# Michaelszeng/GCS-ADMM

Hardware: AMD Instinct MI355X
Metric: admm_iterations_per_sec (higher is better)
Workload: dtype f64; 1 GPU; benchmark4; V=42, E=94, n=2, state_dtype=f64, state_columns=incidence, inner_arithmetic=f64, vertex_program=workgroup, vertex_solves=warm start from the previous iteration's record (csrc/warm_start.h), parallelism=1 GPU

## Files before the change

### gcs_admm_amd/csrc/vertex_wg.h

```cpp
#pragma once
#include <type_traits>

#include "gcs_math.h"
#include "step_args.h"
#include "warm_start.h"

#if defined(__HIP_DEVICE_COMPILE__)
#define WG_DEVICE 1
#else
#define WG_DEVICE 0
#endif

namespace gcs_wg {

using gcs_math::REG_DELTA;
using gcs_math::rcp;
using gcs_math::rcp1;
using gcs_math::rsqrt_nr;
using gcs_math::sqrt_nr;

#ifndef GCS_WG_THREADS
#define GCS_WG_THREADS 256
#endif
constexpr int WG_THREADS = GCS_WG_THREADS;
constexpr int WG_WAVES = WG_THREADS / 64;
constexpr int WG_ITEM_WAVES = WG_WAVES > 1 ? WG_WAVES - 1 : 1;

constexpr bool WG_VM = false;
#if WG_DEVICE
template <bool VM> __device__ __forceinline__ void wg_barrier()
{
    if constexpr (VM) asm volatile("s_waitcnt vmcnt(0)" ::: "memory");
    __syncthreads();
}
template <bool VM> __device__ __forceinline__ void wg_wave_sync()
{
    if constexpr (VM) asm volatile("s_waitcnt vmcnt(0) lgkmcnt(0)" ::: "memory");
    else asm volatile("s_waitcnt lgkmcnt(0)" ::: "memory");
}
__device__ __forceinline__ int wg_tid()
{
    int t = (int)threadIdx.x;
    asm volatile("" : "+v"(t));
    return t;
}
#define WG_FOR(i, cnt) for (int i = gcs_wg::wg_tid(), i##_end = (cnt); i < i##_end; i += gcs_wg::WG_THREADS)
#define WG_FOR_AT(i, cnt, start) for (int i = (gcs_wg::wg_tid() - (start)) & (gcs_wg::WG_THREADS - 1), i##_end = (cnt); i < i##_end; i += gcs_wg::WG_THREADS)
#define WG_SYNC() gcs_wg::wg_barrier<WG_VM>()
#define WG_ONE() if (gcs_wg::wg_tid() == 0)
#define WG_CONE() if (gcs_wg::wg_tid() == gcs_wg::WG_THREADS - 1)
#define WG_CONE2(l) for (int l = gcs_wg::wg_tid() - (gcs_wg::WG_THREADS - 2); l >= 0 && l < 2; l = 2)
#define WG_WAVE0() if (gcs_wg::wg_tid() < 64)
#define WG_FIRST_WAVES(w, cnt) for (int w = gcs_wg::wg_tid() >> 6; w < (cnt); w += gcs_wg::WG_WAVES)
#define WG_ITEM_FOR(q, i, count, PER)                                                                                          \
    for (int t_ = gcs_wg::wg_tid(), w_ = t_ >> 6, l_ = t_ & 63,                                                                \
             n_ = w_ < gcs_wg::WG_ITEM_WAVES ? (((count) - w_ + gcs_wg::WG_ITEM_WAVES - 1) / gcs_wg::WG_ITEM_WAVES) * (PER) : 0;  \
         l_ < n_; l_ += 64)                                                                                                    \
        if (const int qq_ = l_ / (PER), i = l_ - qq_ * (PER), q = w_ + gcs_wg::WG_ITEM_WAVES * qq_; true)
#define WG_REPL_FOR(i, cnt) for (int i = (gcs_wg::wg_tid() >> 6) < gcs_wg::WG_ITEM_WAVES ? (gcs_wg::wg_tid() & 63) : (cnt), i##_end = (cnt); i < i##_end; i += 64)
#define WG_WAVE_SYNC() gcs_wg::wg_wave_sync<WG_VM>()
#define WG_FENCE() asm volatile("" ::: "memory")
#else
#define WG_FENCE() do { } while (0)
#ifdef GCS_WG_REVERSE
#define WG_FOR(i, cnt) for (int i = (cnt) - 1; i >= 0; --i)
#else
#define WG_FOR(i, cnt) for (int i = 0, i##_end = (cnt); i < i##_end; ++i)
#endif
#define WG_FOR_AT(i, cnt, start) WG_FOR(i, ((void)(start), (cnt)))
#define WG_SYNC() do { } while (0)
#define WG_ONE() if (true)
#define WG_CONE() if (true)
#define WG_CONE2(l) for (int l = 0; l < 2; ++l)
#define WG_WAVE0() if (true)
#define WG_FIRST_WAVES(w, cnt) for (int w = 0; w < (cnt); ++w)
#define WG_ITEM_FOR(q, i, count, PER) WG_FOR(t_, (count) * (PER)) if (const int q = t_ / (PER), i = t_ - q * (PER); true)
#define WG_REPL_FOR(i, cnt) WG_FOR(i, cnt)
#define WG_WAVE_SYNC() do { } while (0)
#endif

#if defined(GCS_WG_TIMING) && defined(__HIPCC__)
__device__ unsigned long long g_wg_cycles[64];
__device__ unsigned long long g_wg_counts[64];
__device__ unsigned long long g_wg_wave_cycles[64 * 8];
#endif
#if defined(GCS_WG_TIMING) && WG_DEVICE
__device__ __forceinline__ void wg_stamp(int id, unsigned long long &last)
{
    if (blockIdx.x == 0) {
        const unsigned long long t = __builtin_amdgcn_s_memtime();
        if (threadIdx.x == 0) {
            atomicAdd(&g_wg_cycles[id], t - last);
            atomicAdd(&g_wg_counts[id], 1ull);
        }
        last = t;
    }
}
__device__ __forceinline__ void wg_arrive(int id, unsigned long long last)
{
    if (blockIdx.x == 0) {
        const unsigned long long t = __builtin_amdgcn_s_memtime();
        if ((threadIdx.x & 63) == 0) atomicAdd(&g_wg_wave_cycles[id * 8 + ((threadIdx.x >> 6) & 7)], t - last);
    }
}
#define WG_ARRIVE(id) gcs_wg::wg_arrive(id, wg_last_stamp)
#define WG_STAMP(id) gcs_wg::wg_stamp(id, wg_last_stamp)
#define WG_STAMP_INIT() unsigned long long wg_last_stamp = __builtin_amdgcn_s_memtime()
#else
#define WG_STAMP(id) do { } while (0)
#define WG_ARRIVE(id) do { } while (0)
#define WG_STAMP_INIT() do { } while (0)
#endif

struct Place {
    int off = 0;
    GCS_HD int at(int cnt)
    {
        const int start = off & (WG_THREADS - 1);
        off = (off + cnt + 63) & ~63;
        return start;
    }
};

template <int N> struct WD {
    static constexpr int NW = 2 * N + 1, NX = 2 * N, NB1 = 4 * N + 1, Q = N + 1, NS = N * (N + 1) / 2;
    static constexpr int TA = 2 * NS + 2 * N + 1;
};

constexpr int pad2(int x) { return (x + 1) & ~1; }
template <int N> struct WSoc {
    static constexpr int Q = N + 1;
    static constexpr int SS = 0, LS = Q, WB = 2 * Q, LT = 3 * Q, CV = LT + Q, SU = CV + N, DSSA = SU + N * N, DLSA = DSSA + Q,
                         DSS = DLSA + Q, DLS = DSS + Q, KS = DLS + Q, SIZE = KS + Q;
};
enum { SC_T = 0, SC_DT, SC_DTA, SC_ALPHA, SC_CONEFAIL, SC_C0, SC_ETA, SC_GT, SC_AMAXC, SC_C1C, SC_C2C, SC_AMAXC2, SC_N = 12 };
template <int N> struct WL {
    using D = WD<N>;
    static constexpr int NW = D::NW, NX = D::NX, NB1 = D::NB1;
    static constexpr int CEN = 0, XV = CEN + pad2(N), DX = XV + pad2(NX), NU = DX + pad2(NX), DNU = NU + pad2(2 * NW),
                         BS = DNU + pad2(2 * NW), BSI = BS + pad2(2 * NW * NW), BXS = BSI + pad2(2 * NW * NW),
                         PIVS = BXS + pad2(2 * NW * NX), BG = PIVS + pad2(2 * NW), XBG = BG + pad2(2 * NW), XBX = XBG + pad2(2 * NX),
                         XS = XBX + pad2(2 * NX * NX), RP = XS + pad2(NX * N), VV = RP + pad2(2 * NW), WW = VV + pad2(2 * NW), M = WW + pad2(2 * NW),
                         PIVM = M + pad2(NB1 * NB1), RHS = PIVM + pad2(NB1), SOL = RHS + pad2(NB1),
                         SOC = SOL + pad2(NB1), PQ = SOC + pad2(WSoc<N>::SIZE), PC = PQ + pad2(NX + NW), SC = PC + pad2(NX + NW), RED = SC + pad2(SC_N), FIXED = RED + 3 * 3 * WG_WAVES;
    static constexpr int P = 0, DW = P + pad2(NW), TG = DW + pad2(NW), TF = TG + pad2(NW), LB = TF + pad2(N), KB = LB + 2, DLB = KB + 2,
                         PIV = DLB + 2, G0 = PIV + pad2(NW), GU = G0 + pad2(NW), GX = GU + pad2(NW), TE = GX + pad2(NX),
                         RV = TE + pad2(NW), K = RV + pad2(NW), X = K + pad2(NW * NW), B = X + pad2(NW * NX), ROWS = B + pad2(NW * NW);
    static GCS_HD int unit_stride(int m) { return (ROWS + 12 * m) | 1; }
    static GCS_HD int total(int U, int m) { return FIXED + pad2(U * unit_stride(m)) + pad2(m * N) + pad2(m); }
    static GCS_HD int units_doubles(int U, int m) { return pad2(U * unit_stride(m)); }
};
template <int N> struct WLBox {
    using G = WL<N>;
    using D = WD<N>;
    static constexpr int NW = D::NW, NX = D::NX, NB1 = D::NB1;
    static constexpr int CEN = G::CEN, XV = G::XV, DX = G::DX, NU = G::NU, DNU = G::DNU, BS = G::BS, BSI = G::BSI, BXS = G::BXS, PIVS = G::PIVS,
                         BG = G::BG, XBG = G::XBG, XBX = G::XBX, XS = G::XS, RP = G::RP, VV = G::VV, WW = G::WW, M = G::M, PIVM = G::PIVM,
                         RHS = G::RHS, SOL = G::SOL, SOC = G::SOC, PQ = G::PQ, PC = G::PC, SC = G::SC, RED = G::RED, FIXED = G::FIXED;
    static constexpr int P = G::P, DW = G::DW, TG = G::TG, TF = G::TF, LB = G::LB, KB = G::KB, DLB = G::DLB, G0 = G::G0, GU = G::GU, GX = G::GX,
                         TE = G::TE, RV = G::RV;
    static constexpr int KD = G::K, KY = KD + pad2(NX), KYY = KY + pad2(NX), XD = KYY + 2, XY = XD + pad2(NX),
                         BD = XY + pad2(NX), BW = BD + pad2(NX), BRS = BW + pad2(NW), BQ = BRS + 2, ROWS = BQ + pad2(NX);
    static GCS_HD int unit_stride(int m) { return (ROWS + 12 * m) | 1; }
    static GCS_HD int total(int U, int m) { return FIXED + pad2(U * unit_stride(m)) + pad2(m * N) + pad2(m); }
    static GCS_HD int units_doubles(int U, int m) { return pad2(U * unit_stride(m)); }
};
template <int N> GCS_HD int wg_lds_doubles(int U, int m, bool box = false) { return box ? WLBox<N>::total(U, m) : WL<N>::total(U, m); }
constexpr int WG_MAX_N = 8;
inline bool wg_has_box(int n) { return n == 3 || n == 6; }
inline int wg_lds_doubles_n(int n, int U, int m, bool box = false)
{
    box = box && wg_has_box(n);
    switch (n) {
    case 1: return wg_lds_doubles<1>(U, m);
    case 2: return wg_lds_doubles<2>(U, m);
    case 3: return wg_lds_doubles<3>(U, m, box);
    case 4: return wg_lds_doubles<4>(U, m);
    case 5: return wg_lds_doubles<5>(U, m);
    case 6: return wg_lds_doubles<6>(U, m, box);
    case 7: return wg_lds_doubles<7>(U, m);
    default: return wg_lds_doubles<8>(U, m);
    }
}

struct alignas(8) WgF2 { float a, b; };

template <class T> struct WgArgs : gcsadmm_k::StepArgs<T> {
    int n_vtx;
    const int *vtx;
    const double *prox_q = nullptr, *prox_c = nullptr;
    const int *order = nullptr;
    int *unit_iters = nullptr;
};

struct Red3 { double mn, s1, s2; };

#if WG_DEVICE
template <int SH> __device__ __forceinline__ double dpp_row_shr(double x, double ident)
{
    const int ilo = __double2loint(ident), ihi = __double2hiint(ident);
    const int lo = __builtin_amdgcn_update_dpp(ilo, __double2loint(x), 0x110 + SH, 0xf, 0xf, false);
    const int hi = __builtin_amdgcn_update_dpp(ihi, __double2hiint(x), 0x110 + SH, 0xf, 0xf, false);
    return __hiloint2double(hi, lo);
}
__device__ __forceinline__ double lane_bcast(double x, int lane)
{
    return __hiloint2double(__builtin_amdgcn_readlane(__double2hiint(x), lane), __builtin_amdgcn_readlane(__double2loint(x), lane));
}
#endif

GCS_HD double wg_uniform(double x)
{
#if WG_DEVICE
    return __hiloint2double(__builtin_amdgcn_readfirstlane(__double2hiint(x)), __builtin_amdgcn_readfirstlane(__double2loint(x)));
#else
    return x;
#endif
}
GCS_HD int wg_uniform(int x)
{
#if WG_DEVICE
    return __builtin_amdgcn_readfirstlane(x);
#else
    return x;
#endif
}

template <bool VM = false> GCS_HD Red3 wg_reduce(Red3 v, double *red, int &phase)
{
#if WG_DEVICE
    v.mn = fmin(v.mn, dpp_row_shr<1>(v.mn, 1e300)); v.s1 += dpp_row_shr<1>(v.s1, 0.0); v.s2 += dpp_row_shr<1>(v.s2, 0.0);
    v.mn = fmin(v.mn, dpp_row_shr<2>(v.mn, 1e300)); v.s1 += dpp_row_shr<2>(v.s1, 0.0); v.s2 += dpp_row_shr<2>(v.s2, 0.0);
    v.mn = fmin(v.mn, dpp_row_shr<4>(v.mn, 1e300)); v.s1 += dpp_row_shr<4>(v.s1, 0.0); v.s2 += dpp_row_shr<4>(v.s2, 0.0);
    v.mn = fmin(v.mn, dpp_row_shr<8>(v.mn, 1e300)); v.s1 += dpp_row_shr<8>(v.s1, 0.0); v.s2 += dpp_row_shr<8>(v.s2, 0.0);
    Red3 w;
    w.mn = fmin(fmin(lane_bcast(v.mn, 15), lane_bcast(v.mn, 31)), fmin(lane_bcast(v.mn, 47), lane_bcast(v.mn, 63)));
    w.s1 = (lane_bcast(v.s1, 15) + lane_bcast(v.s1, 31)) + (lane_bcast(v.s1, 47) + lane_bcast(v.s1, 63));
    w.s2 = (lane_bcast(v.s2, 15) + lane_bcast(v.s2, 31)) + (lane_bcast(v.s2, 47) + lane_bcast(v.s2, 63));
    double *buf = red + phase * (3 * WG_WAVES);
    phase = phase == 2 ? 0 : phase + 1;
    const int wave = (int)threadIdx.x >> 6;
    if (((int)threadIdx.x & 63) == 0) { buf[wave * 3 + 0] = w.mn; buf[wave * 3 + 1] = w.s1; buf[wave * 3 + 2] = w.s2; }
    wg_barrier<VM>();
    Red3 r{buf[0], buf[1], buf[2]};
#pragma unroll
    for (int q = 1; q < WG_WAVES; ++q) { r.mn = fmin(r.mn, buf[3 * q]); r.s1 += buf[3 * q + 1]; r.s2 += buf[3 * q + 2]; }
    return r;
#else
    (void)red; (void)phase;
    return v;
#endif
}

GCS_HD void tri_decode(int t, int &r, int &c)
{
    r = (int)((sqrtf(8.0f * (float)t + 1.0f) - 1.0f) * 0.5f);
    if ((r + 1) * (r + 2) / 2 <= t) ++r;
    if (r * (r + 1) / 2 > t) --r;
    c = t - r * (r + 1) / 2;
}

GCS_HD int fdiv(int x, float inv) { return (int)(((float)x + 0.5f) * inv); }

GCS_HD constexpr int pki(int i, int j) { return i * (i + 1) / 2 + j; }

template <int DIM> GCS_HD void wave_ldl(double *Mq, double *rd)
{
    static_assert(DIM <= 64, "one row per lane");
#if WG_DEVICE
    const int lane = wg_tid() & 63, row = lane < DIM ? lane : DIM - 1;
    double a[DIM];
#pragma unroll
    for (int j = 0; j < DIM; ++j) a[j] = Mq[row * DIM + j];
    const double od = Mq[row * DIM + row];
    double myr = 0.0;
#pragma unroll
    for (int k = 0; k < DIM; ++k) {
        const double dk = lane_bcast(a[k], k);
        const double odk = lane_bcast(od, k);
        const double rk = rcp(gcs_math::pivot_floor(dk, odk)), col = a[k], l = col * rk;
        a[k] = l;
        if (lane == k) myr = rk;
#pragma unroll
        for (int j = k + 1; j < DIM; ++j) a[j] -= l * lane_bcast(col, j);
    }
    if (lane < DIM) {
#pragma unroll
        for (int j = 0; j < DIM - 1; ++j) Mq[lane * DIM + j] = a[j];
        rd[lane] = myr;
    }
#else
    double od[DIM], col[DIM];
    for (int k = 0; k < DIM; ++k) od[k] = Mq[k * DIM + k];
    for (int k = 0; k < DIM; ++k) {
        const double rk = rcp(gcs_math::pivot_floor(Mq[k * DIM + k], od[k]));
        rd[k] = rk;
        for (int i = k + 1; i < DIM; ++i) col[i] = Mq[i * DIM + k];
        for (int i = k + 1; i < DIM; ++i) {
            const double l = col[i] * rk;
            Mq[i * DIM + k] = l;
            for (int j = k + 1; j <= i; ++j) Mq[i * DIM + j] -= l * col[j];
        }
    }
#endif
}

template <int DIM> GCS_HD void wave_ldl_solve(const double *Mq, const double *rd, const double *b, double *x)
{
#if WG_DEVICE
    const int lane = wg_tid() & 63, row = lane < DIM ? lane : DIM - 1;
// ... 144 lines not shown
    const int WUS = WR::unit_stride(m);
    double dtm = 0.0;
    Place pl0;
    WG_FOR_AT(t, d * NW, pl0.at(d * NW)) {
        const int e = t / NW, w = t - e * NW, edge = a.inc_edge[lo + e];
        const bool out = e >= d_in;
        const int inc = gcsadmm_k::state_column(a, lo, e, edge, out);
        double *un = UN(e + 1);
        const double Tw = gcsadmm_k::consensus_target(a, w, edge, inc, mu_scale);
        int slot = -1;
        if (w == 2 * N) slot = 2 * N;
        else if (out) slot = w;
        else if (w < N) { un[W::TF + w] = Tw; un[W::TG + N + w] = 0.0; }
        else slot = w - N;
        if (slot >= 0) {
            un[W::TG + slot] = Tw;
            if (wrec) dtm = fmax(dtm, fabs(Tw - wrec[WR::UNITS + (e + 1) * WUS + WR::TG + slot]));
        }
    }
    WG_FOR_AT(t, m * N, pl0.at(m * N)) PA[t] = a.poly_A[(size_t)p0 * N + t];
    WG_FOR_AT(j, m + N, pl0.at(m + N)) {
        if (j < m) PA[pad2(m * N) + j] = a.poly_bc[p0 + j];
        else sm[W::CEN + (j - m)] = a.center[(size_t)v * N + (j - m)];
    }
    if (prox) {
        WG_FOR(k, NX + NW) {
            sm[W::PQ + k] = a.prox_q[(size_t)v * (NX + NW) + k];
            sm[W::PC + k] = a.prox_c[(size_t)v * (NX + NW) + k];
        }
    }
    bool use_warm = false;
    double mu_ref = gcs_ws::WS_COLD_REF, ws_dT = -1.0;
    if (wrec) {
        const Red3 rt = wg_reduce<WG_VM>(Red3{-dtm, 0.0, 0.0}, sm + W::RED, red_phase);
        const bool comparable = wg_uniform((int)(wrec[0] == 1.0 && wrec[1] == rho)) != 0;
        ws_dT = wg_uniform(comparable ? -rt.mn * rho : -1.0);
        use_warm = wg_uniform((int)(comparable && ws_dT <= gcs_ws::ws_theta(wrec))) != 0;
        if (use_warm) mu_ref = wg_uniform(fmax(gcs_ws::WS_MU_MIN, gcs_ws::WS_KAPPA * ws_dT));
    }
    const bool ws_started_warm = use_warm;
    const float inv_R2 = 1.0f / (float)(R / 2);

    WG_STAMP(0);
    auto gval = [&](const double *un, int u, int k, bool wk) {
        double g = un[W::G0 + k];
        if (wk) {
            g += un[W::GU + k];
            if (u == 0 && k < 2 * N) g += k < N ? -SOC[SO::KS + 1 + k] : SOC[SO::KS + 1 + (k - N)];
        }
        return g;
    };
    auto te_tasks = [&](Place &pl, bool wk) {
        WG_FOR_AT(t, d * NW, pl.at(d * NW)) {
            const int u = 1 + t / NW, i = t - (u - 1) * NW;
            double *un = UN(u);
            double s = 0;
            if constexpr (BOX) {
                double wg = 0;
#pragma unroll
                for (int k = 0; k < NW; ++k) wg += un[W::BW + k] * gval(un, u, k, wk);
                s = -(un[W::BRS] * un[W::BW + i]) * wg;
                if (i < 2 * N) s -= un[W::BD + i] * gval(un, u, i, wk);
            } else {
#pragma unroll
                for (int k = 0; k < NW; ++k) s -= un[W::B + i * NW + k] * gval(un, u, k, wk);
            }
            un[W::TE + i] = s;
        }
    };
    auto bg_tasks = [&](Place &pl) {
        WG_FOR_AT(t, 2 * NW, pl.at(2 * NW)) {
            const int s = t / NW, i = t - s * NW;
            double acc = 0;
#pragma unroll 4
            for (int u = side_lo(s); u <= side_hi(s); ++u) acc += UN(u)[W::TE + i];
            sm[W::BG + t] = acc;
        }
        WG_FOR_AT(t, 2 * NX, pl.at(2 * NX)) {
            const int part = t / NX, c = t - part * NX, h = c / N;
            const int ulo = part ? 1 + d / 2 : 1, uhi = part ? d : d / 2;
            double acc = 0;
#pragma unroll 2
            for (int u = ulo; u <= uhi; ++u) {
                const double *un = UN(u);
                if constexpr (BOX) acc += un[W::XD + c] * un[W::TE + c] + un[W::XY + c] * un[W::TE + 2 * N];
                else {
#pragma unroll
                    for (int k = 0; k < N; ++k) acc += un[W::X + (h * N + k) * NX + c] * un[W::TE + h * N + k];
                    acc += un[W::X + 2 * N * NX + c] * un[W::TE + 2 * N];
                }
            }
            sm[W::XBG + t] = acc;
        }
    };
    auto v_tasks = [&](Place &pl) {
        WG_FOR_AT(t, 2 * NW, pl.at(2 * NW)) {
            const int s = t / NW, i = t - s * NW;
            const double *Bsi = sm + W::BSI + s * NW * NW;
            double acc = 0;
#pragma unroll
            for (int k = 0; k < NW; ++k) acc += Bsi[i * NW + k] * (sm[W::RP + s * NW + k] - sm[W::BG + s * NW + k]);
            sm[W::VV + t] = acc;
        }
    };
    auto rhs_tasks = [&](Place &pl, bool wk) {
        const double *u0 = UN(0);
        auto base_z = [&](int i) { return -gval(u0, 0, i, wk) - sm[W::VV + i] - sm[W::VV + NW + i]; };
        WG_FOR_AT(q, NX, pl.at(NX)) {
            double r = -REG_DELTA * sm[W::XV + q] - sm[W::XBG + q] - sm[W::XBG + NX + q];
            if (prox) r -= sm[W::PQ + q] * (sm[W::XV + q] + CEN[q < N ? q : q - N] - sm[W::PC + q]);
            if (wk) r -= sm[W::SOL + q];
            for (int s = 0; s < 2; ++s) {
                const double *BXs = sm + W::BXS + s * NW * NX;
#pragma unroll
                for (int i = 0; i < NW; ++i) r -= BXs[i * NX + q] * sm[W::VV + s * NW + i];
            }
            sm[W::RHS + q] = r;
        }
        WG_FOR_AT(k, N, pl.at(N))
            sm[W::RHS + NX + k] = base_z(k) + SOC[SO::CV + k] * SC[SC_GT] * rcp(SC[SC_C0]);
        WG_FOR_AT(k, N, pl.at(N))
            sm[W::RHS + NX + N + k] = base_z(k) + base_z(N + k);
        WG_FOR_AT(k, 1, pl.at(1)) sm[W::RHS + NX + 2 * N + k] = base_z(2 * N);
    };
    auto solve_head = [&](bool wk) {
        {
            Place pl;
            te_tasks(pl, wk);
            if (wk) {
                WG_FOR_AT(q, NX, pl.at(NX)) {
                    double acc = 0;
#pragma unroll 4
                    for (int u = 0; u <= d; ++u) acc += UN(u)[W::GX + q];
                    sm[W::SOL + q] = acc;
                }
            }
        }
        WG_ARRIVE(30);
        WG_SYNC();
        WG_STAMP(30);
        { Place pl; bg_tasks(pl); }
        WG_ARRIVE(31);
        WG_SYNC();
        WG_STAMP(31);
        { Place pl; v_tasks(pl); }
        WG_ARRIVE(32);
        WG_SYNC();
        WG_STAMP(32);
        { Place pl; rhs_tasks(pl, wk); }
        WG_ARRIVE(33);
        WG_SYNC();
        WG_STAMP(33);
    };
    auto cone_dir = [&](int dt_slot, bool wk, double (&xs)[Q], double (&dl)[Q]) {
        const double *u0 = UN(0);
        double wb[Q], ys[Q];
        xs[0] = SC[dt_slot];
#pragma unroll
        for (int k = 0; k < N; ++k) xs[1 + k] = u0[W::DW + k] - u0[W::DW + N + k];
#pragma unroll
        for (int k = 0; k < Q; ++k) wb[k] = SOC[SO::WB + k];
        soc_apply_W2<Q>(wb, SC[SC_ETA], xs, ys);
#pragma unroll
        for (int k = 0; k < Q; ++k) dl[k] = (wk ? SOC[SO::KS + k] : 0.0) - SOC[SO::LS + k] - ys[k];
    };
    auto solve_tail = [&](int dt_slot, bool wk) {
        WG_WAVE0() wave_ldl_solve<NB1>(sm + W::M, sm + W::PIVM, sm + W::RHS, sm + W::SOL);
        WG_ARRIVE(34);
        WG_SYNC();
        WG_STAMP(34);
        auto dzeta = [&](int i) { return i < N ? sm[W::SOL + NX + i] + sm[W::SOL + NX + N + i] : sm[W::SOL + NX + i]; };
        Place plw;
        WG_FOR_AT(t, 2 * NW, plw.at(2 * NW)) {
            const int s = t / NW, i = t - s * NW;
            const double *BXs = sm + W::BXS + s * NW * NX;
            double acc = dzeta(i) + (sm[W::RP + t] - sm[W::BG + t]);
#pragma unroll
            for (int c = 0; c < NX; ++c) acc += BXs[i * NX + c] * sm[W::SOL + c];
            sm[W::WW + t] = acc;
        }
        WG_FOR_AT(t, NX + NW + 1, plw.at(NX + NW + 1)) {
            if (t < NX) sm[W::DX + t] = sm[W::SOL + t];
            else if (t < NX + NW) UN(0)[W::DW + (t - NX)] = dzeta(t - NX);
            else {
                double acc = -SC[SC_GT];
#pragma unroll
                for (int k = 0; k < N; ++k) acc -= SOC[SO::CV + k] * sm[W::SOL + NX + k];
                SC[dt_slot] = acc * rcp(SC[SC_C0]);
            }
        }
        WG_ARRIVE(36);
        WG_SYNC();
        WG_STAMP(36);
        auto cone_bounds = [&](int l) {
            const int oDS = wk ? SO::DSS : SO::DSSA, oDL = wk ? SO::DLS : SO::DLSA;
            double xs[Q], dl[Q], bs[Q], dr[Q];
            cone_dir(dt_slot, wk, xs, dl);
            double c1c = 0, c2c = 0;
#pragma unroll
            for (int k = 0; k < Q; ++k) {
                const double sk = SOC[SO::SS + k], lk = SOC[SO::LS + k];
                SOC[oDS + k] = xs[k]; SOC[oDL + k] = dl[k];
                c1c += sk * dl[k] + lk * xs[k];
                c2c += xs[k] * dl[k];
                bs[k] = l == 1 ? lk : sk; dr[k] = l == 1 ? dl[k] : xs[k];
            }
            SC[SC_C1C] = c1c; SC[SC_C2C] = c2c;
            SC[l == 1 ? SC_AMAXC2 : SC_AMAXC] = gcs_math::soc_max_step<Q>(bs, dr);
            if (l == 2) SC[SC_AMAXC2] = gcs_math::soc_max_step<Q>(SOC + SO::LS, dl);
        };
        if constexpr (CONE_PAIR) { WG_CONE2(l) cone_bounds(l); }
        else { WG_CONE() cone_bounds(2); }
        WG_REPL_FOR(t, 2 * NW) {
            const int s = t / NW, i = t - s * NW;
            const double *Bsi = sm + W::BSI + s * NW * NW;
            double acc = 0;
#pragma unroll
            for (int k = 0; k < NW; ++k) acc += Bsi[i * NW + k] * sm[W::WW + s * NW + k];
            sm[W::DNU + t] = acc;
        }
        WG_WAVE_SYNC();
        WG_ITEM_FOR(q, i, d, NW) {
            const int u = 1 + q;
            double *un = UN(u);
            double acc = -gval(un, u, i, wk) + sm[W::DNU + side_of(u) * NW + i];
            if constexpr (BOX) {
                if (i < 2 * N) acc -= un[W::XD + i] * sm[W::DX + i];
                else {
#pragma unroll
                    for (int c = 0; c < NX; ++c) acc -= un[W::XY + c] * sm[W::DX + c];
                }
            } else if (i < 2 * N) {
                const int h = i / N;
#pragma unroll
                for (int k = 0; k < N; ++k) acc -= un[W::X + i * NX + h * N + k] * sm[W::DX + h * N + k];
            } else {
#pragma unroll
                for (int c = 0; c < NX; ++c) acc -= un[W::X + i * NX + c] * sm[W::DX + c];
            }
            un[W::RV + i] = acc;
        }
        WG_WAVE_SYNC();
        WG_ITEM_FOR(q, i, d, NW) {
            double *un = UN(1 + q);
            double acc = 0;
            if constexpr (BOX) {
                double wr = 0;
#pragma unroll
                for (int k = 0; k < NW; ++k) wr += un[W::BW + k] * un[W::RV + k];
                acc = (un[W::BRS] * un[W::BW + i]) * wr;
                if (i < 2 * N) acc += un[W::BD + i] * un[W::RV + i];
            } else {
#pragma unroll
                for (int k = 0; k < NW; ++k) acc += un[W::B + i * NW + k] * un[W::RV + k];
            }
            un[W::DW + i] = acc;
        }
        WG_ARRIVE(39);
        WG_SYNC();
        WG_STAMP(39);
    };

    int status = -1, it = 0, it_total = 0, stalled = 0;
    bool saved = false, init_pending = true;
#define WG_FAIL_OR_RESTART()                                                                                                   \
    {                                                                                                                          \
        if (!use_warm) break;                                                                                                  \
        it_total += it; it = -1;                                                                                               \
        use_warm = false; mu_ref = gcs_ws::WS_COLD_REF; init_pending = true;                                                   \
        WG_SYNC();                                                                                                             \
        continue;                                                                                                              \
    }
    for (it = 0;; ++it) {
    if (init_pending) {
        init_pending = false; stalled = 0; saved = false;
        Place pls;
        if (use_warm) {
            const double *wu = wrec + WR::UNITS;
            WG_FOR_AT(t, U * NW, pls.at(U * NW)) {
                const int u = t / NW, k = t - u * NW;
                UN(u)[W::P + k] = wu[u * WUS + WR::P + k];
            }
            WG_FOR_AT(t, U * (R / 2), pls.at(U * (R / 2))) {
                const int u = fdiv(t, inv_R2), r2 = t - u * (R / 2);
                const WgF2 v = reinterpret_cast<const WgF2 *>(wu + u * WUS + WR::LAM)[r2];
                UN(u)[oLAM + 2 * r2] = (double)v.a; UN(u)[oLAM + 2 * r2 + 1] = (double)v.b;
            }
            WG_FOR_AT(t, 2 * U, pls.at(2 * U)) UN(t >> 1)[W::LB + (t & 1)] = wu[(t >> 1) * WUS + WR::LB + (t & 1)];
            WG_FOR_AT(k, NX + 2 * NW, pls.at(NX + 2 * NW)) {
                if (k < NX) sm[W::XV + k] = wrec[WR::XV + k];
                else sm[W::NU + (k - NX)] = wrec[WR::NU + (k - NX)];
            }
        } else {
            WG_FOR_AT(t, U * NW, pls.at(U * NW)) {
                const int u = t / NW, k = t - u * NW;
                double val = 0.0;
                if (k == 2 * N) val = u == 0 ? 0.5 : 0.5 / (double)(side_of(u) ? d_out : d_in);
                UN(u)[W::P + k] = val;
            }
            WG_FOR_AT(k, NX + 2 * NW, pls.at(NX + 2 * NW)) {
                if (k < NX) sm[W::XV + k] = 0.0;
                else sm[W::NU + (k - NX)] = 0.0;
            }
            WG_ONE() {
                SC[SC_T] = 1.0;
                SOC[SO::LS] = 1.0;
                for (int k = 1; k < Q; ++k) SOC[SO::LS + k] = 0.0;
            }
        }
        WG_SYNC();
    }
        const bool first_warm = use_warm && it == 0;
        double acc = 0.0; int bad = 0;
        Place plr;
        WG_ROWS_BEGIN(plr)
            const double is = rcp1(s);
            if (it == 0 && !use_warm) un[oLAM + ro] = is;
            const double l = un[oLAM + ro];
            un[oR1 + ro] = l * is;
            acc += s * l;
            if (!(s > 0.0)) bad = 1;
        WG_ROWS_END()
        WG_FOR_AT(u, U, plr.at(U)) {
            double *un = UN(u);
            const double yy = un[W::P + 2 * N], s5 = yy, s6 = 1.0 - yy;
            if (it == 0 && !use_warm) { un[W::LB] = rcp1(s5); un[W::LB + 1] = rcp1(s6); }
            acc += s5 * un[W::LB] + s6 * un[W::LB + 1];
            if (!(s5 > 0.0) || !(s6 > 0.0)) bad = 1;
        }
        WG_FOR_AT(tg, U * NW, plr.at(U * NW)) {
            const int u = tg / NW, k = tg - u * NW;
            double *un = UN(u);
            const double *p = un + W::P;
            double g;
            if (u == 0) {
                g = sm[W::NU + k] + sm[W::NU + NW + k] + REG_DELTA * p[k];
                if (prox) {
                    const double *qz = sm + W::PQ + NX, *cz = sm + W::PC + NX;
                    const double yy = p[2 * N];
                    if (k < 2 * N) g += qz[k] * (p[k] + yy * CEN[k < N ? k : k - N] - cz[k]);
                    else {
                        g += qz[2 * N] * (yy - cz[2 * N]);
#pragma unroll
                        for (int c = 0; c < 2 * N; ++c) g += CEN[c < N ? c : c - N] * qz[c] * (p[c] + yy * CEN[c < N ? c : c - N] - cz[c]);
                    }
                }
            }
            else {
                const bool out = side_of(u);
                const double *tg_ = un + W::TG, *nu = sm + W::NU + (out ? NW : 0);
                const double yy = p[2 * N];
                if (k < N) g = rho * (p[k] + yy * CEN[k] - tg_[k]);
                else if (k < 2 * N) g = out ? rho * (p[k] + yy * CEN[k - N] - tg_[k]) : 0.0;
                else {
                    g = rho * (yy - tg_[2 * N]) + a.eps_edge;
#pragma unroll
                    for (int c = 0; c < N; ++c) {
                        g += CEN[c] * rho * (p[c] + yy * CEN[c] - tg_[c]);
                        if (out) g += CEN[c] * rho * (p[N + c] + yy * CEN[c] - tg_[N + c]);
                    }
                }
                g += REG_DELTA * p[k] - nu[k];
            }
            un[W::G0 + k] = g;
        }
        WG_CONE() {
            const double *u0 = UN(0);
            if (first_warm) {
                double uu = 0;
                for (int k = 0; k < N; ++k) { const double uk = u0[W::P + k] - u0[W::P + N + k]; uu += uk * uk; }
                const double tn = 0.5 * (mu_ref + sqrt_nr(mu_ref * mu_ref + 4.0 * uu)), itn = rcp(tn);
                SC[SC_T] = tn;
                SOC[SO::LS] = 1.0;
                for (int k = 0; k < N; ++k) SOC[SO::LS + 1 + k] = -(u0[W::P + k] - u0[W::P + N + k]) * itn;
            }
            SOC[SO::SS] = SC[SC_T];
            for (int k = 0; k < N; ++k) SOC[SO::SS + 1 + k] = u0[W::P + k] - u0[W::P + N + k];
            for (int k = 0; k < Q; ++k) acc += SOC[SO::SS + k] * SOC[SO::LS + k];
            if (!gcs_math::soc_interior<Q>(SOC + SO::SS)) bad = 1;
        }
        WG_ARRIVE(1);
        const Red3 r0 = wg_reduce<WG_VM>(Red3{bad ? -1.0 : 1.0, acc, 0.0}, sm + W::RED, red_phase);
        WG_STAMP(1);
        const double gap = wg_uniform(r0.s1);
        const double mu = wg_uniform(r0.mn < 0.0 ? 0.0 / 0.0 : gap * inv_deg);
        WG_FENCE();
        if (wrec != nullptr && !saved && it >= 1 && mu <= gcs_ws::WS_SAVE * mu_ref) {
            saved = true;
            double *wu = wrec + WR::UNITS;
            Place plv;
            WG_FOR_AT(t, U * NW, plv.at(U * NW)) {
                const int u = t / NW, k = t - u * NW;
                wu[u * WUS + WR::P + k] = UN(u)[W::P + k];
                if (u > 0) wu[u * WUS + WR::TG + k] = UN(u)[W::TG + k];
            }
            WG_FOR_AT(t, U * (R / 2), plv.at(U * (R / 2))) {
                const int u = fdiv(t, inv_R2), r2 = t - u * (R / 2);
                WgF2 v; v.a = (float)UN(u)[oLAM + 2 * r2]; v.b = (float)UN(u)[oLAM + 2 * r2 + 1];
                reinterpret_cast<WgF2 *>(wu + u * WUS + WR::LAM)[r2] = v;
            }
            WG_FOR_AT(t, 2 * U, plv.at(2 * U)) wu[(t >> 1) * WUS + WR::LB + (t & 1)] = UN(t >> 1)[W::LB + (t & 1)];
            WG_FOR_AT(k, NX + 2 * NW, plv.at(NX + 2 * NW)) {
                if (k < NX) wrec[WR::XV + k] = sm[W::XV + k];
                else wrec[WR::NU + (k - NX)] = sm[W::NU + (k - NX)];
            }
            WG_ONE() { wrec[0] = 1.0; wrec[1] = rho; }
        }
        WG_FENCE();
        {
            const bool conv = gcs_math::mu_converged(mu, a.ipm_tol, stalled, first_warm);
            bool stop = conv;
            status = conv ? ((use_warm && !(mu <= a.ipm_tol)) ? -7 : 0) : -1;
            if (!(mu > 0.0)) { stop = true; status = -3; }
            if (!stop && it >= a.ipm_max_iter) { stop = true; status = -1; }
            if (stop) { if (status == 0) break; WG_FAIL_OR_RESTART(); }
        }

        WG_CONE() {
            double wb[Q], eta = 1.0;
            if (!gcs_math::soc_scaling_wb<Q>(SOC + SO::SS, SOC + SO::LS, wb, eta)) SC[SC_CONEFAIL] = 1.0;
            else {
                SC[SC_CONEFAIL] = 0.0; SC[SC_ETA] = eta;
                const double ieta = rcp(eta), ie2 = ieta * ieta;
#pragma unroll
                for (int i = 0; i < Q; ++i) SOC[SO::WB + i] = wb[i];
                {
                    double ls[Q], lt[Q];
#pragma unroll
                    for (int i = 0; i < Q; ++i) ls[i] = SOC[SO::LS + i];
                    soc_apply_W<Q>(wb, eta, ls, lt);
#pragma unroll
                    for (int i = 0; i < Q; ++i) SOC[SO::LT + i] = lt[i];
                }
                const double den = 2.0 * wb[0] * wb[0] - 1.0, g2 = 2.0 * rcp(den);
                SC[SC_C0] = ie2 * den;
                for (int k = 0; k < N; ++k) {
                    SOC[SO::CV + k] = -ie2 * 2.0 * wb[0] * wb[1 + k];
                    for (int l = 0; l < N; ++l) SOC[SO::SU + k * N + l] = ie2 * ((k == l ? 1.0 : 0.0) - g2 * wb[1 + k] * wb[1 + l]);
                }
            }
            SC[SC_GT] = 1.0;
        }
        Place pla;
        const int sK_ = pla.at(BOX ? U * 2 * N : U * 2 * NS), sKy_ = BOX ? 0 : pla.at(U * 2 * N), sKyy_ = pla.at(U);
        (void)sKy_;
        if constexpr (BOX) {
            WG_FOR_AT(t, U * 2 * N, sK_) {
                const int u = t / (2 * N), ik = t - u * (2 * N), i = ik / N, k = ik - i * N;
                double *un = UN(u);
                const double *Da = un + oR1, *Db = Da + m2;
                const bool blk = u > 0, out = blk && side_of(u);
                const double dp = Da[i * m + k] + Db[i * m + k], dn = Da[i * m + k + N] + Db[i * m + k + N];
                const double bp = BC[k], bn = -BC[k + N];
                double sk = dp + dn;
                sk += REG_DELTA; if (blk && (i == 0 || out)) sk += rho; if (prox) sk += sm[W::PQ + NX + i * N + k];
                un[W::KD + ik] = sk;
                un[W::XD + ik] = -(Db[i * m + k] + Db[i * m + k + N]);
                double sy = -(dp * bp) - dn * bn;
                if (blk && (i == 0 || out)) sy += rho * CEN[k];
                if (prox) sy += sm[W::PQ + NX + i * N + k] * CEN[k];
                un[W::KY + ik] = sy;
                un[W::XY + ik] = Db[i * m + k] * bp + Db[i * m + k + N] * bn;
            }
        } else {
            WG_FOR_AT(t, U * 2 * NS, sK_) {
                const int u = t / (2 * NS), q = t - u * (2 * NS), i = q / NS, pq = q - i * NS;
                double *un = UN(u);
                double *K = un + W::K, *X = un + W::X;
                const double *Da = un + oR1, *Db = Da + m2;
                const bool blk = u > 0, out = blk && side_of(u);
                int k, l;
                if constexpr (N == 2) { k = pq > 0; l = pq > 1; }
                else tri_decode(pq, k, l);
                double sk = 0, sx = 0;
    #pragma unroll 4
                for (int j = 0; j < m; ++j) {
                    const double aa = A[j * N + k] * A[j * N + l];
                    sk += (Da[i * m + j] + Db[i * m + j]) * aa;
                    sx += Db[i * m + j] * aa;
                }
                if (k == l) { sk += REG_DELTA; if (blk && (i == 0 || out)) sk += rho; if (prox) sk += sm[W::PQ + NX + i * N + k]; }
                K[(i * N + k) * NW + i * N + l] = sk; K[(i * N + l) * NW + i * N + k] = sk;
                X[(i * N + k) * NX + i * N + l] = -sx; X[(i * N + l) * NX + i * N + k] = -sx;
                const int o = (1 - i) * N;
                K[(i * N + k) * NW + o + l] = 0.0; K[(i * N + l) * NW + o + k] = 0.0;
                X[(i * N + k) * NX + o + l] = 0.0; X[(i * N + l) * NX + o + k] = 0.0;
            }
            WG_FOR_AT(t, U * 2 * N, sKy_) {
                const int u = t / (2 * N), ik = t - u * (2 * N), i = ik / N, k = ik - i * N;
                double *un = UN(u);
                const double *Da = un + oR1, *Db = Da + m2;
                const bool blk = u > 0, out = blk && side_of(u);
                double sk = 0, sx = 0;
    #pragma unroll 4
                for (int j = 0; j < m; ++j) {
                    const double ba = BC[j] * A[j * N + k];
                    sk -= (Da[i * m + j] + Db[i * m + j]) * ba;
                    sx += Db[i * m + j] * ba;
                }
                if (blk && (i == 0 || out)) sk += rho * CEN[k];
                if (prox) sk += sm[W::PQ + NX + i * N + k] * CEN[k];
                un[W::K + (i * N + k) * NW + 2 * N] = sk; un[W::K + 2 * N * NW + i * N + k] = sk;
                un[W::X + 2 * N * NX + i * N + k] = sx;
            }
        }
        WG_FOR_AT(u, U, sKyy_) {
            double *un = UN(u);
            const double *Da = un + oR1, *Db = Da + m2;
            const bool blk = u > 0, out = blk && side_of(u);
            double sk = 0;
#pragma unroll 4
            for (int j = 0; j < m2; ++j) { const double b = BC[j >= m ? j - m : j]; sk += (Da[j] + Db[j]) * b * b; }
            const double yy = un[W::P + 2 * N];
            sk += un[W::LB] * rcp1(yy) + un[W::LB + 1] * rcp1(1.0 - yy) + REG_DELTA;
            if (blk) {
                double cc = 0;
#pragma unroll
                for (int k = 0; k < N; ++k) cc += CEN[k] * CEN[k];
                sk += rho * (1.0 + (out ? 2.0 : 1.0) * cc);
            }
            if (prox) {
                sk += sm[W::PQ + NX + 2 * N];
#pragma unroll
                for (int k = 0; k < 2 * N; ++k) sk += sm[W::PQ + NX + k] * CEN[k < N ? k : k - N] * CEN[k < N ? k : k - N];
            }
            if constexpr (BOX) un[W::KYY] = sk; else un[W::K + 2 * N * NW + 2 * N] = sk;
        }
        WG_ARRIVE(2);
        WG_SYNC();
        WG_STAMP(2);
        if (wg_uniform(SC[SC_CONEFAIL]) != 0.0) {
            status = gcs_math::boundary_status(mu, a.ipm_tol, use_warm);
            if (status == 0) break;
            WG_FAIL_OR_RESTART();
        }

        WG_FOR(t, 2 * d) {
            const int u = 1 + (t >> 1), h = t & 1;
            double *un = UN(u);
            if constexpr (BOX) {
                double ch = 0;
#pragma unroll
                for (int r = 0; r < N; ++r) {
                    const double dd = un[W::KD + h * N + r], kr = un[W::KY + h * N + r];
                    const double inv = rsqrt_nr(dd), lr = kr * inv;
                    un[W::BD + h * N + r] = inv * inv;
                    un[W::BW + h * N + r] = lr * inv;
                    ch += lr * lr;
                }
                un[W::RV + h] = ch;
            } else {
            double a[NS], kv[N], pv[N];
#pragma unroll
            for (int i = 0; i < N; ++i) {
                kv[i] = un[W::K + (h * N + i) * NW + 2 * N];
#pragma unroll
                for (int j = 0; j <= i; ++j) a[pki(i, j)] = un[W::K + (h * N + i) * NW + h * N + j];
            }
#pragma unroll
            for (int j = 0; j < N; ++j) {
                const double od = a[pki(j, j)];
                double dj = od;
#pragma unroll
                for (int k = 0; k < j; ++k) dj -= a[pki(j, k)] * a[pki(j, k)];
                const double inv = rsqrt_nr(gcs_math::pivot_floor(dj, od));
                pv[j] = inv;
#pragma unroll
                for (int i = j + 1; i < N; ++i) {
                    double sij = a[pki(i, j)];
#pragma unroll
                    for (int k = 0; k < j; ++k) sij -= a[pki(i, k)] * a[pki(j, k)];
                    a[pki(i, j)] = sij * inv;
                }
            }
            double (&li)[NS] = a;
#pragma unroll
            for (int c = 0; c < N; ++c)
#pragma unroll
                for (int i = c; i < N; ++i) {
                    double sx = (i == c) ? 1.0 : 0.0;
#pragma unroll
                    for (int k = c; k < i; ++k) sx -= a[pki(i, k)] * li[pki(k, c)];
                    li[pki(i, c)] = sx * pv[i];
                }
#pragma unroll
            for (int r = 0; r < N; ++r)
#pragma unroll
                for (int c = 0; c <= r; ++c) {
// ... 452 lines not shown
```

Measured before the change: 9829 iterations/s.

## Fold solve-tail back-substitution into precomputed operators and drop an intermediate barrier

Removes the intermediate WW vector stage in the vertex solve tail. The dual-step and per-unit direction updates are now computed directly from the LDL solution, using composed operators (BSI times dzeta plus a BS-based term, and B/K or BW/BQ per unit) together with precomputed VV/TE offsets. The cone direction's dt is recomputed inline from the solution with a cached reciprocal of C0, so one workgroup barrier and one wave-sync pass disappear. This relies on the precomputed matrices and offsets being algebraically equivalent to the old chained products, and it adds per-thread arithmetic in exchange for fewer synchronisation points.

New measurement: 10160 iterations/s (median of 6 runs). +3.3%, better.

```diff
diff --git a/gcs_admm_amd/csrc/vertex_wg.h b/gcs_admm_amd/csrc/vertex_wg.h
--- a/gcs_admm_amd/csrc/vertex_wg.h
+++ b/gcs_admm_amd/csrc/vertex_wg.h
@@ -133,14 +133,14 @@
     static constexpr int SS = 0, LS = Q, WB = 2 * Q, LT = 3 * Q, CV = LT + Q, SU = CV + N, DSSA = SU + N * N, DLSA = DSSA + Q,
                          DSS = DLSA + Q, DLS = DSS + Q, KS = DLS + Q, SIZE = KS + Q;
 };
-enum { SC_T = 0, SC_DT, SC_DTA, SC_ALPHA, SC_CONEFAIL, SC_C0, SC_ETA, SC_GT, SC_AMAXC, SC_C1C, SC_C2C, SC_AMAXC2, SC_N = 12 };
+enum { SC_T = 0, SC_DT, SC_DTA, SC_ALPHA, SC_CONEFAIL, SC_C0, SC_ETA, SC_GT, SC_AMAXC, SC_C1C, SC_C2C, SC_AMAXC2, SC_IC0, SC_N = 13 };
 template <int N> struct WL {
     using D = WD<N>;
     static constexpr int NW = D::NW, NX = D::NX, NB1 = D::NB1;
     static constexpr int CEN = 0, XV = CEN + pad2(N), DX = XV + pad2(NX), NU = DX + pad2(NX), DNU = NU + pad2(2 * NW),
                          BS = DNU + pad2(2 * NW), BSI = BS + pad2(2 * NW * NW), BXS = BSI + pad2(2 * NW * NW),
                          PIVS = BXS + pad2(2 * NW * NX), BG = PIVS + pad2(2 * NW), XBG = BG + pad2(2 * NW), XBX = XBG + pad2(2 * NX),
-                         XS = XBX + pad2(2 * NX * NX), RP = XS + pad2(NX * N), VV = RP + pad2(2 * NW), WW = VV + pad2(2 * NW), M = WW + pad2(2 * NW),
+                         XS = XBX + pad2(2 * NX * NX), RP = XS + pad2(NX * N), VV = RP + pad2(2 * NW), M = VV + pad2(2 * NW),
                          PIVM = M + pad2(NB1 * NB1), RHS = PIVM + pad2(NB1), SOL = RHS + pad2(NB1),
                          SOC = SOL + pad2(NB1), PQ = SOC + pad2(WSoc<N>::SIZE), PC = PQ + pad2(NX + NW), SC = PC + pad2(NX + NW), RED = SC + pad2(SC_N), FIXED = RED + 3 * 3 * WG_WAVES;
     static constexpr int P = 0, DW = P + pad2(NW), TG = DW + pad2(NW), TF = TG + pad2(NW), LB = TF + pad2(N), KB = LB + 2, DLB = KB + 2,
@@ -155,7 +155,7 @@
     using D = WD<N>;
     static constexpr int NW = D::NW, NX = D::NX, NB1 = D::NB1;
     static constexpr int CEN = G::CEN, XV = G::XV, DX = G::DX, NU = G::NU, DNU = G::DNU, BS = G::BS, BSI = G::BSI, BXS = G::BXS, PIVS = G::PIVS,
-                         BG = G::BG, XBG = G::XBG, XBX = G::XBX, XS = G::XS, RP = G::RP, VV = G::VV, WW = G::WW, M = G::M, PIVM = G::PIVM,
+                         BG = G::BG, XBG = G::XBG, XBX = G::XBX, XS = G::XS, RP = G::RP, VV = G::VV, M = G::M, PIVM = G::PIVM,
                          RHS = G::RHS, SOL = G::SOL, SOC = G::SOC, PQ = G::PQ, PC = G::PC, SC = G::SC, RED = G::RED, FIXED = G::FIXED;
     static constexpr int P = G::P, DW = G::DW, TG = G::TG, TF = G::TF, LB = G::LB, KB = G::KB, DLB = G::DLB, G0 = G::G0, GU = G::GU, GX = G::GX,
                          TE = G::TE, RV = G::RV;
@@ -606,12 +606,16 @@
         WG_SYNC();
         WG_STAMP(33);
     };
+    auto dzeta = [&](int i) { return i < N ? sm[W::SOL + NX + i] + sm[W::SOL + NX + N + i] : sm[W::SOL + NX + i]; };
     auto cone_dir = [&](int dt_slot, bool wk, double (&xs)[Q], double (&dl)[Q]) {
-        const double *u0 = UN(0);
         double wb[Q], ys[Q];
-        xs[0] = SC[dt_slot];
-#pragma unroll
-        for (int k = 0; k < N; ++k) xs[1 + k] = u0[W::DW + k] - u0[W::DW + N + k];
+        double acc = -SC[SC_GT];
+#pragma unroll
+        for (int k = 0; k < N; ++k) acc -= SOC[SO::CV + k] * sm[W::SOL + NX + k];
+        xs[0] = acc * SC[SC_IC0];
+        SC[dt_slot] = xs[0];
+#pragma unroll
+        for (int k = 0; k < N; ++k) xs[1 + k] = dzeta(k) - dzeta(N + k);
 #pragma unroll
         for (int k = 0; k < Q; ++k) wb[k] = SOC[SO::WB + k];
         soc_apply_W2<Q>(wb, SC[SC_ETA], xs, ys);
@@ -623,29 +627,10 @@
         WG_ARRIVE(34);
         WG_SYNC();
         WG_STAMP(34);
-        auto dzeta = [&](int i) { return i < N ? sm[W::SOL + NX + i] + sm[W::SOL + NX + N + i] : sm[W::SOL + NX + i]; };
-        Place plw;
-        WG_FOR_AT(t, 2 * NW, plw.at(2 * NW)) {
-            const int s = t / NW, i = t - s * NW;
-            const double *BXs = sm + W::BXS + s * NW * NX;
-            double acc = dzeta(i) + (sm[W::RP + t] - sm[W::BG + t]);
-#pragma unroll
-            for (int c = 0; c < NX; ++c) acc += BXs[i * NX + c] * sm[W::SOL + c];
-            sm[W::WW + t] = acc;
-        }
-        WG_FOR_AT(t, NX + NW + 1, plw.at(NX + NW + 1)) {
+        WG_FOR_AT(t, NX + NW, WG_THREADS - 64) {
             if (t < NX) sm[W::DX + t] = sm[W::SOL + t];
-            else if (t < NX + NW) UN(0)[W::DW + (t - NX)] = dzeta(t - NX);
-            else {
-                double acc = -SC[SC_GT];
-#pragma unroll
-                for (int k = 0; k < N; ++k) acc -= SOC[SO::CV + k] * sm[W::SOL + NX + k];
-                SC[dt_slot] = acc * rcp(SC[SC_C0]);
-            }
-        }
-        WG_ARRIVE(36);
-        WG_SYNC();
-        WG_STAMP(36);
+            else UN(0)[W::DW + (t - NX)] = dzeta(t - NX);
+        }
         auto cone_bounds = [&](int l) {
             const int oDS = wk ? SO::DSS : SO::DSSA, oDL = wk ? SO::DLS : SO::DLSA;
             double xs[Q], dl[Q], bs[Q], dr[Q];
@@ -667,46 +652,35 @@
         else { WG_CONE() cone_bounds(2); }
         WG_REPL_FOR(t, 2 * NW) {
             const int s = t / NW, i = t - s * NW;
-            const double *Bsi = sm + W::BSI + s * NW * NW;
-            double acc = 0;
-#pragma unroll
-            for (int k = 0; k < NW; ++k) acc += Bsi[i * NW + k] * sm[W::WW + s * NW + k];
-            sm[W::DNU + t] = acc;
+            const double *Bsi = sm + W::BSI + s * NW * NW, *Ys = sm + W::BS + s * NW * NW;
+            double acc = sm[W::VV + t], acc2 = 0;
+#pragma unroll
+            for (int k = 0; k < NW; ++k) acc += Bsi[i * NW + k] * dzeta(k);
+#pragma unroll
+            for (int c = 0; c < NX; ++c) acc2 += Ys[i * NX + c] * sm[W::SOL + c];
+            sm[W::DNU + t] = acc + acc2;
         }
         WG_WAVE_SYNC();
         WG_ITEM_FOR(q, i, d, NW) {
             const int u = 1 + q;
             double *un = UN(u);
-            double acc = -gval(un, u, i, wk) + sm[W::DNU + side_of(u) * NW + i];
+            const double *dnu = sm + W::DNU + side_of(u) * NW, *dx = sm + W::SOL;
+            double acc = un[W::TE + i];
             if constexpr (BOX) {
-                if (i < 2 * N) acc -= un[W::XD + i] * sm[W::DX + i];
-                else {
-#pragma unroll
-                    for (int c = 0; c < NX; ++c) acc -= un[W::XY + c] * sm[W::DX + c];
-                }
-            } else if (i < 2 * N) {
-                const int h = i / N;
-#pragma unroll
-                for (int k = 0; k < N; ++k) acc -= un[W::X + i * NX + h * N + k] * sm[W::DX + h * N + k];
+                double wn = 0, qx = 0;
+#pragma unroll
+                for (int k = 0; k < NW; ++k) wn += un[W::BW + k] * dnu[k];
+#pragma unroll
+                for (int c = 0; c < NX; ++c) qx += un[W::BQ + c] * dx[c];
+                acc += (un[W::BRS] * un[W::BW + i]) * (wn - qx);
+                if (i < 2 * N) acc += un[W::BD + i] * (dnu[i] - un[W::XD + i] * dx[i]);
             } else {
-#pragma unroll
-                for (int c = 0; c < NX; ++c) acc -= un[W::X + i * NX + c] * sm[W::DX + c];
-            }
-            un[W::RV + i] = acc;
-        }
-        WG_WAVE_SYNC();
-        WG_ITEM_FOR(q, i, d, NW) {
-            double *un = UN(1 + q);
-            double acc = 0;
-            if constexpr (BOX) {
-                double wr = 0;
-#pragma unroll
-                for (int k = 0; k < NW; ++k) wr += un[W::BW + k] * un[W::RV + k];
-                acc = (un[W::BRS] * un[W::BW + i]) * wr;
-                if (i < 2 * N) acc += un[W::BD + i] * un[W::RV + i];
-            } else {
-#pragma unroll
-                for (int k = 0; k < NW; ++k) acc += un[W::B + i * NW + k] * un[W::RV + k];
+                double acc2 = 0;
+#pragma unroll
+                for (int k = 0; k < NW; ++k) acc += un[W::B + i * NW + k] * dnu[k];
+#pragma unroll
+                for (int c = 0; c < NX; ++c) acc2 += un[W::K + i * NX + c] * dx[c];
+                acc -= acc2;
             }
             un[W::DW + i] = acc;
         }
@@ -887,7 +861,7 @@
                     for (int i = 0; i < Q; ++i) SOC[SO::LT + i] = lt[i];
                 }
                 const double den = 2.0 * wb[0] * wb[0] - 1.0, g2 = 2.0 * rcp(den);
-                SC[SC_C0] = ie2 * den;
+                SC[SC_C0] = ie2 * den; SC[SC_IC0] = rcp(ie2 * den);
                 for (int k = 0; k < N; ++k) {
                     SOC[SO::CV + k] = -ie2 * 2.0 * wb[0] * wb[1 + k];
                     for (int l = 0; l < N; ++l) SOC[SO::SU + k * N + l] = ie2 * ((k == l ? 1.0 : 0.0) - g2 * wb[1 + k] * wb[1 + l]);
```
